# andrewhou1/GeomConsistentFR

Measured on AMD Instinct MI355X. Metric: ray_steps_per_sec, higher is better.
Workload: dtype f64+f32

## Files before the change

### geomconsistentfr_amd/csrc/gcfr_device.hpp

```cpp
#pragma once

#include <hip/hip_runtime.h>
#include <stdint.h>

namespace gcfr {

constexpr float kEps4 = 0.0001f;
constexpr float kMaskedDistance = 1000000.0f;

constexpr int kBufferRsrcWord3 = 0x00020000;

__device__ inline __amdgpu_buffer_rsrc_t make_rsrc(const void *p, int bytes)
{
    return __builtin_amdgcn_make_buffer_rsrc(const_cast<void *>(p), 0, bytes, kBufferRsrcWord3);
}
__device__ inline float buf_load_f32(__amdgpu_buffer_rsrc_t r, int byte_off)
{
    return __builtin_bit_cast(float, __builtin_amdgcn_raw_buffer_load_b32(r, byte_off, 0, 0));
}
__device__ inline uint32_t buf_load_u8(__amdgpu_buffer_rsrc_t r, int byte_off)
{
    return __builtin_amdgcn_raw_buffer_load_b8(r, byte_off, 0, 0);
}

struct Box {
    float x_lo, x_hi, y_lo, y_hi;
};
__device__ __host__ inline Box image_box(int H, int W)
{
    return Box{-(W / 2.0f), W - W / 2.0f - 1.0f, 1.0f - H / 2.0f, H / 2.0f};
}

struct LightCase {
    int xcase, ycase;
};
__device__ inline LightCase classify_light(float Cx, float Cy, const Box &bx)
{
    LightCase lc;
    lc.xcase = (Cx < bx.x_lo) ? 0 : (Cx <= bx.x_hi ? 1 : 2);
    lc.ycase = (Cy < bx.y_lo) ? 0 : (Cy <= bx.y_hi ? 1 : 2);
    return lc;
}

__device__ inline void end_point(float x, float y, float Cx, float Cy, const Box &bx, LightCase lc,
                                 float &Ex, float &Ey)
{
    const float m = (Cy - y) / ((Cx - x) + kEps4);
    const float ic = Cy - m * Cx;
    float ex, ey;
    if (lc.xcase == 1) {
        if (lc.ycase == 1) {
            ex = Cx;
            ey = Cy;
        } else {
            const float yb = (lc.ycase == 0) ? bx.y_lo : bx.y_hi;
            ex = (yb - ic) / (m + kEps4);
            ey = yb;
        }
    } else {
        const float xb = (lc.xcase == 0) ? bx.x_lo : bx.x_hi;
        const float Xy = m * xb + ic;
        if (lc.ycase == 1) {
            ex = xb;
            ey = Xy;
        } else {
            const float yb = (lc.ycase == 0) ? bx.y_lo : bx.y_hi;
            const float Yx = (yb - ic) / (m + kEps4);
            const float b = (Yx >= bx.x_lo && Yx <= bx.x_hi) ? 1.0f : 0.0f;
            const float nb = 1.0f - b;
            ex = Yx * b + xb * nb;
            ey = yb * b + Xy * nb;
        }
    }
    ex = (ex < bx.x_lo) ? bx.x_lo : ex;
    ex = (ex > bx.x_hi) ? bx.x_hi : ex;
    ey = (ey < bx.y_lo) ? bx.y_lo : ey;
    ey = (ey > bx.y_hi) ? bx.y_hi : ey;
    Ex = ex;
    Ey = ey;
}

__device__ inline float sqrt_rn_normal(float x)
{
#ifdef GCFR_R04_FIXED_COST
    return __builtin_sqrtf(x);
#endif
    const float s = __builtin_amdgcn_sqrtf(x);
    const int si = __builtin_bit_cast(int, s);
    const float s_dn = __builtin_bit_cast(float, si - 1), s_up = __builtin_bit_cast(float, si + 1);
    const float e_dn = __builtin_fmaf(-s_dn, s, x), e_up = __builtin_fmaf(-s_up, s, x);
    float o = (e_dn <= 0.0f) ? s_dn : s;
    o = (e_up > 0.0f) ? s_up : o;
    return o;
}

__device__ inline float norm3_torch(float a, float b, float c)
{
    return __builtin_sqrtf(__builtin_fmaf(c, c, __builtin_fmaf(b, b, a * a)));
}

__device__ inline float exp_neg(float d)
{
    const float x = -((d > 200.0f) ? 200.0f : d);
    const float kL2eHi = 1.44269502e+0f, kL2eLo = 1.92596299e-8f;
    const float t = x * kL2eHi;
    const float lo = __builtin_fmaf(x, kL2eLo, __builtin_fmaf(x, kL2eHi, -t));
    const float r = __builtin_amdgcn_exp2f(t);
    return __builtin_fmaf(r, lo * 0.693147182f, r);
}
__device__ inline float shadow_transfer(float d)
{
#ifdef GCFR_R04_FIXED_COST
    {
        const float e = expf(-d);
        const float onepe = 1.0f + e;
        return (-4.0f * e) / (onepe * onepe) + 1.0f;
    }
#endif
    const float e = exp_neg(d);
    const float onepe = 1.0f + e;
    const float q = onepe * onepe;
    float rq = __builtin_amdgcn_rcpf(q);
    rq = __builtin_fmaf(__builtin_fmaf(-q, rq, 1.0f), rq, rq);
    return (-4.0f * e) * rq + 1.0f;
}

struct Shaded {
    float w, full, fin;
};
__device__ inline float inv_norm3_clamped(float a, float b, float c)
{
    const float s2 = __builtin_fmaf(c, c, __builtin_fmaf(b, b, a * a));
    const float r = __builtin_amdgcn_rsqf(s2);
    const float r1 = r * __builtin_fmaf(-0.5f * s2 * r, r, 1.5f);
    return s2 > 1e-24f ? r1 : 1e12f;
}
__device__ inline float lambert_dot(float x, float y, float zb, float nx, float ny, float nz, float Cx, float Cy, float Cz)
{
    const float lx = Cx - x, ly = Cy - y, lz = Cz - zb;
#ifdef GCFR_R04_FIXED_COST
    {
        float ln = norm3_torch(lx, ly, lz);
        ln = ln > 1e-12f ? ln : 1e-12f;
        const float ux = lx / ln, uy = ly / ln, uz = lz / ln;
        float nn = norm3_torch(nx, ny, nz);
        nn = nn > 1e-12f ? nn : 1e-12f;
        const float n0 = nx / nn, n1 = ny / nn, n2 = nz / nn;
        return (n0 * ux + n1 * uy) + n2 * uz;
    }
#endif
    const float rl = inv_norm3_clamped(lx, ly, lz);
    const float ux = lx * rl, uy = ly * rl, uz = lz * rl;
    const float rn = inv_norm3_clamped(nx, ny, nz);
    const float n0 = nx * rn, n1 = ny * rn, n2 = nz * rn;
    return (n0 * ux + n1 * uy) + n2 * uz;
}

__device__ inline Shaded shade_pixel(float x, float y, float zb, float nx, float ny, float nz, float Cx,
                                     float Cy, float Cz, float amb, float intensity, float min_dist)
{
    const float dot = lambert_dot(x, y, zb, nx, ny, nz, Cx, Cy, Cz);
    Shaded o;
    o.full = amb + intensity * (dot > 0.0f ? dot : 0.0f);
    o.w = shadow_transfer(min_dist);
    o.fin = o.w * o.full + (1.0f - o.w) * amb;
    return o;
}

struct NormalsArgs {
    const float *depth;
    float *normals;
    const float *grad_normals;
    float *grad_depth;
    int32_t H, W;
    double fx, fy, cx, cy;
    float z_offset;
    int32_t negate_y;
    double inv_fx, inv_fy;
};
inline void set_focal(NormalsArgs &a, double fx, double fy)
{
    a.fx = fx;
    a.fy = fy;
    a.inv_fx = 1.0 / fx;
    a.inv_fy = 1.0 / fy;
}

__device__ constexpr double kSobelU[3][3] = {{-0.125, 0.0, 0.125}, {-0.25, 0.0, 0.25}, {-0.125, 0.0, 0.125}};
__device__ constexpr double kSobelV[3][3] = {{-0.125, -0.25, -0.125}, {0.0, 0.0, 0.0}, {0.125, 0.25, 0.125}};

struct Grad3 {
    double du[3], dv[3];
};

__device__ inline double fast_rcp64(double x)
{
    double r = __builtin_amdgcn_rcp(x);
    r = __builtin_fma(r, __builtin_fma(-x, r, 1.0), r);
    r = __builtin_fma(r, __builtin_fma(-x, r, 1.0), r);
    return r;
}

__device__ inline double fast_sqrt64(double x)
{
    double y = __builtin_amdgcn_rsq(x);
    double g = x * y, h = 0.5 * y;
    double e = __builtin_fma(-h, g, 0.5);
    g = __builtin_fma(g, e, g);
    h = __builtin_fma(h, e, h);
    e = __builtin_fma(-h, g, 0.5);
    g = __builtin_fma(g, e, g);
    return g;
}

__device__ inline Grad3 point_gradients(const NormalsArgs &a, const float *z, int r, int c)
{
    Grad3 g = {{0.0, 0.0, 0.0}, {0.0, 0.0, 0.0}};
    int rr[3], cc[3];
    double ax[3], ay[3];
#pragma unroll
    for (int j = 0; j < 3; ++j) {
        rr[j] = min(max(r + j - 1, 0), a.H - 1);
        cc[j] = min(max(c + j - 1, 0), a.W - 1);
        ax[j] = ((double)cc[j] - a.cx) * a.inv_fx;
        ay[j] = ((double)rr[j] - a.cy) * a.inv_fy;
    }
#pragma unroll
    for (int dr = -1; dr <= 1; ++dr) {
#pragma unroll
        for (int dc = -1; dc <= 1; ++dc) {
            const double d = (double)(z[(size_t)rr[dr + 1] * a.W + cc[dc + 1]] + a.z_offset);
            const double ku = kSobelU[dr + 1][dc + 1], kv = kSobelV[dr + 1][dc + 1];
            if (ku == 0.0 && kv == 0.0) {
                g.du[2] = __builtin_fma(0.0, d, g.du[2]);
                continue;
            }
            const double X = ax[dc + 1] * d, Y = ay[dr + 1] * d;
            if (ku != 0.0) {
                g.du[0] = __builtin_fma(ku, X, g.du[0]);
                g.du[1] = __builtin_fma(ku, Y, g.du[1]);
                g.du[2] = __builtin_fma(ku, d, g.du[2]);
            }
            if (kv != 0.0) {
                g.dv[0] = __builtin_fma(kv, X, g.dv[0]);
                g.dv[1] = __builtin_fma(kv, Y, g.dv[1]);
                g.dv[2] = __builtin_fma(kv, d, g.dv[2]);
            }
        }
    }
    return g;
}

__device__ inline double fast_rsqrt64(double x)
{
    const double y = __builtin_amdgcn_rsq(x);
    const double g = x * y, h = 0.5 * y;
    return __builtin_fma(y, __builtin_fma(-h, g, 0.5), y);
}

__device__ inline void unit_normal(const NormalsArgs &a, const float *z, int r, int c, float (&n)[3])
{
#ifdef GCFR_R04_FIXED_COST
    {
        const Grad3 g = point_gradients(a, z, r, c);
        const double nx = __builtin_fma(g.du[1], g.dv[2], -(g.du[2] * g.dv[1]));
        const double ny = __builtin_fma(g.du[2], g.dv[0], -(g.du[0] * g.dv[2]));
        const double nz = __builtin_fma(g.du[0], g.dv[1], -(g.du[1] * g.dv[0]));
        const double n2sum = __builtin_fma(nz, nz, __builtin_fma(ny, ny, nx * nx));
        double nn = n2sum > 1e-24 ? fast_sqrt64(n2sum) : 1e-12;
        nn = nn > 1e-12 ? nn : 1e-12;
        const double inv = fast_rcp64(nn);
        n[0] = (float)(nx * inv);
        n[1] = (float)(a.negate_y ? -(ny * inv) : (ny * inv));
        n[2] = (float)(nz * inv);
        return;
    }
#endif
    const int W = a.W;
    const bool has_l = c > 0, has_r = c < W - 1, has_u = r > 0, has_d = r < a.H - 1;
    const __amdgpu_buffer_rsrc_t zr = make_rsrc(z, a.H * W * 4);
    const int b11 = (r * W + c) << 2, W4 = W << 2;
    const int bu = has_u ? b11 - W4 : b11, bd = has_d ? b11 + W4 : b11;
    const int ol = has_l ? 4 : 0, orr = has_r ? 4 : 0;
    const float off = a.z_offset;
    const float D11 = buf_load_f32(zr, b11) + off;
    const float e00 = (buf_load_f32(zr, bu - ol) + off) - D11, e01 = (buf_load_f32(zr, bu) + off) - D11, e02 = (buf_load_f32(zr, bu + orr) + off) - D11;
    const float e10 = (buf_load_f32(zr, b11 - ol) + off) - D11, e12 = (buf_load_f32(zr, b11 + orr) + off) - D11;
    const float e20 = (buf_load_f32(zr, bd - ol) + off) - D11, e21 = (buf_load_f32(zr, bd) + off) - D11, e22 = (buf_load_f32(zr, bd + orr) + off) - D11;
    const float h0 = e02 - e00, h1 = e12 - e10, h2 = e22 - e20;
    const float g0 = e20 - e00, g1 = e21 - e01, g2 = e22 - e02;
    const float a8 = __builtin_fmaf(2.0f, h1, h0 + h2), b8 = __builtin_fmaf(2.0f, g1, g0 + g2);
    const float er = __builtin_fmaf(2.0f, e12, e02 + e22), el = __builtin_fmaf(2.0f, e10, e00 + e20);
    const float eb = __builtin_fmaf(2.0f, e21, e20 + e22), et = __builtin_fmaf(2.0f, e01, e00 + e02);
    const float s_x = (has_r ? er : 0.0f) + (has_l ? el : 0.0f), s_y = (has_d ? eb : 0.0f) + (has_u ? et : 0.0f);
    const float v_y = (has_d ? h2 : 0.0f) - (has_u ? h0 : 0.0f), v_x = (has_r ? g2 : 0.0f) - (has_l ? g0 : 0.0f);
    const float Dx = (has_l && has_r) ? D11 : 0.5f * D11, Dy = (has_u && has_d) ? D11 : 0.5f * D11;
    const double inv_fx = a.inv_fx, inv_fy = a.inv_fy;
    const double px = inv_fx * __builtin_fma(0.125, (double)s_x, (double)Dx), py = (0.125 * inv_fy) * (double)v_y;
    const double qx = (0.125 * inv_fx) * (double)v_x, qy = inv_fy * __builtin_fma(0.125, (double)s_y, (double)Dy);
    const double da = 0.125 * (double)a8, db = 0.125 * (double)b8;
    const double mx = __builtin_fma(da, qx, -(db * px)), my = __builtin_fma(da, qy, -(db * py));
    const double ax = ((double)c - a.cx) * inv_fx, ay = ((double)r - a.cy) * inv_fy;
    const double nx = -my, ny = mx;
    const double nz = __builtin_fma(ax, my, -(ay * mx)) + __builtin_fma(px, qy, -(py * qx));
    const double n2sum = __builtin_fma(nz, nz, __builtin_fma(ny, ny, nx * nx));
    const double inv = n2sum > 1e-24 ? fast_rsqrt64(n2sum) : 1e12;
    n[0] = (float)(nx * inv);
    n[1] = (float)(a.negate_y ? -(ny * inv) : (ny * inv));
    n[2] = (float)(nz * inv);
}

struct StencilGrad {
    double ddu[3], ddv[3];
};
__device__ inline StencilGrad normals_bwd_terms(const NormalsArgs &a, const float *z, int r, int c, double g0,
                                                double g1_in, double g2)
{
#pragma clang fp contract(fast)
    const Grad3 g = point_gradients(a, z, r, c);
    const double cx_ = g.du[1] * g.dv[2] - g.du[2] * g.dv[1];
    const double cy_ = g.du[2] * g.dv[0] - g.du[0] * g.dv[2];
    const double cz_ = g.du[0] * g.dv[1] - g.du[1] * g.dv[0];
    const double c2sum = cx_ * cx_ + cy_ * cy_ + cz_ * cz_;
    const double nrm = c2sum > 1e-24 ? fast_sqrt64(c2sum) : 0.0;
    const double nn = nrm > 1e-12 ? nrm : 1e-12;
    const double inv_nn = fast_rcp64(nn);
    const double n0 = cx_ * inv_nn, n1 = cy_ * inv_nn, n2 = cz_ * inv_nn;
    const double g1 = a.negate_y ? -g1_in : g1_in;
    double dc0, dc1, dc2;
    if (nrm > 1e-12) {
        const double ng = n0 * g0 + n1 * g1 + n2 * g2;
        dc0 = (g0 - n0 * ng) * inv_nn;
        dc1 = (g1 - n1 * ng) * inv_nn;
        dc2 = (g2 - n2 * ng) * inv_nn;
    } else {
        dc0 = g0 * inv_nn;
        dc1 = g1 * inv_nn;
        dc2 = g2 * inv_nn;
    }
    StencilGrad o;
    o.ddu[0] = g.dv[1] * dc2 - g.dv[2] * dc1;
    o.ddu[1] = g.dv[2] * dc0 - g.dv[0] * dc2;
    o.ddu[2] = g.dv[0] * dc1 - g.dv[1] * dc0;
    o.ddv[0] = dc1 * g.du[2] - dc2 * g.du[1];
    o.ddv[1] = dc2 * g.du[0] - dc0 * g.du[2];
    o.ddv[2] = dc0 * g.du[1] - dc1 * g.du[0];
    return o;
}

template <class Pred>
__device__ inline void normals_bwd_scatter(const NormalsArgs &a, const StencilGrad &sg, float *gz, int r, int c, Pred want)
{
#pragma clang fp contract(fast)
    const double inv_fx = a.inv_fx, inv_fy = a.inv_fy;
#pragma unroll
    for (int dr = -1; dr <= 1; ++dr) {
#pragma unroll
        for (int dc = -1; dc <= 1; ++dc) {
            const double ku = kSobelU[dr + 1][dc + 1], kv = kSobelV[dr + 1][dc + 1];
            if (ku == 0.0 && kv == 0.0)
                continue;
            if (!want(dr, dc))
                continue;
            const int rr = min(max(r + dr, 0), a.H - 1), cc = min(max(c + dc, 0), a.W - 1);
            const double ax = ((double)cc - a.cx) * inv_fx, ay = ((double)rr - a.cy) * inv_fy;
            const double dPx = ku * sg.ddu[0] + kv * sg.ddv[0];
            const double dPy = ku * sg.ddu[1] + kv * sg.ddv[1];
            const double dPz = ku * sg.ddu[2] + kv * sg.ddv[2];
#ifdef GCFR_ATOMIC_HOOK
            GCFR_ATOMIC_HOOK(gz + (size_t)rr * a.W + cc);
#endif
            atomicAdd(gz + (size_t)rr * a.W + cc, (float)(ax * dPx + ay * dPy + dPz));
        }
    }
}

__device__ inline void normals_bwd_pixel(const NormalsArgs &a, const float *z, float *gz, int r, int c,
                                         double g0, double g1_in, double g2)
{
    const StencilGrad sg = normals_bwd_terms(a, z, r, c, g0, g1_in, g2);
    normals_bwd_scatter(a, sg, gz, r, c, [](int, int) { return true; });
}

}
```

### geomconsistentfr_amd/csrc/gcfr_march.hpp

```cpp
#pragma once

#include "gcfr_device.hpp"
#include "gcfr_mutants.hpp"

#include "../../include/gcfr.h"

#include <atomic>
#include <cstddef>
#include <type_traits>

namespace gcfr {

struct ShadowArgs {
    const float *depth;
    const uint8_t *mask;
    const float *light_pt;
    const double *t_table;
    float *min_dist;
    int32_t *argmin;
    int32_t mask_batch, L, H, W, N;
    int32_t tiles_x, tiles_per_image;
    float bonus, bx_lo, bx_hi, by_lo, by_hi;
};

// ... 801 lines not shown
        ++cnt_since_body;
#endif
        const bool dead = OWN && (lane_last < 0);
        bool none = true;
#pragma unroll
        for (int j = 0; j < DEPTH; ++j) {
            none = none && (cm[j] == 0);
            any_masked |= (cm[j] == 0);
        }
        none = none || dead;
        bool run_body = __builtin_amdgcn_ballot_w64(!none) != 0ull;
        if (LAZY) {
            run_body = __builtin_amdgcn_ballot_w64(!none && !cw_in) != 0ull;
        } else if (run_body && use_zb) {
            const bool cannot_win = bound_cw(cz, ta64, tb64, k0);
            run_body = __builtin_amdgcn_ballot_w64(!none && !cannot_win) != 0ull;
            if (TRAIL)
                all_lazy = !run_body && __builtin_amdgcn_ballot_w64(!((cannot_win && GCFR_M(18, true, (bestS < safeS))) || (lane_last < k0))) == 0ull;
        }
#ifndef GCFR_INFER_BODY_CHUNK
#define GCFR_INFER_BODY_CHUNK 1
#endif
        constexpr int GCFR_BODY_CHUNK = KSPLIT ? DEPTH : (WANT_ARGMIN && DEPTH >= 2 ? 2 : GCFR_INFER_BODY_CHUNK);
        if (run_body) {
          GCFR_COUNT(kCntBodies, 1);
#ifdef GCFR_COUNTERS
          if (!cnt_had_body)
              cnt[kCntVisitsBeforeFirstBody] += cnt_since_body - 1;
          cnt_had_body = 1;
          cnt_since_body = 0;
#endif
#ifdef GCFR_COUNTERS
#pragma unroll
          for (int j = 0; j < DEPTH; ++j)
              cnt[kCntLaneSamples] += (unsigned)__builtin_popcountll(__builtin_amdgcn_ballot_w64(cm[j] != 0));
#endif
#pragma unroll
          for (int h0 = 0; h0 < DEPTH; h0 += GCFR_BODY_CHUNK) {
            double ux[DEPTH], uy[DEPTH], fxd[DEPTH], fyd[DEPTH];
            f32x4 qv[DEPTH];
#pragma unroll
            for (int j = h0; j < h0 + GCFR_BODY_CHUNK && j < DEPTH; ++j) {
                constexpr bool CARRIED = FUSE_SHADE || WANT_ARGMIN;
                const double tj = (CARRIED && j == 0) ? ta64 : ((CARRIED && j == DEPTH - 1) ? tb64 : (double)tt[clampk(k0 + j)]);
                const double sx = x64 + tj * dx64, sy = y64 + tj * dy64;
                ux[j] = (sx + halfW) - 0.0001;
                uy[j] = (halfH - sy) - 0.0001;
                fxd[j] = __builtin_floor(ux[j]);
                fyd[j] = __builtin_floor(uy[j]);
                const int fx = (int)fxd[j], fy = (int)fyd[j];
                const int texel = __mul24(fy, Wp) + fx;
                qv[j] = __builtin_bit_cast(
                    f32x4, __builtin_amdgcn_raw_buffer_load_b128(qr, (texel << 4) + quad_origin, 0, 0));
            }
#pragma unroll
            for (int j = h0; j < h0 + GCFR_BODY_CHUNK && j < DEPTH; ++j)
                eval_sample(clampk(k0 + j), (cm[j] == 0) || dead, ux[j], uy[j], fxd[j], fyd[j], qv[j]);
          }
        }
        return finish_check(k0, tn64, check_finished);
    };
    auto group = [&](int k0, const Prefetched &cur, Prefetched &nxt, bool check_finished) -> bool {
        const double ta64 = tc0, tb64 = tc3;
        tc0 = tq[0];
        tc3 = tq[DEPTH - 1];
        prefetch(nxt);
        load_tq(k0 + 2 * DEPTH);
        return consume(k0, cur.m, cur.z, ta64, tb64, tc0, check_finished, std::false_type{}, false);
    };

    auto group_lds = [&](int k0, bool check_finished) -> bool {
        const double ta64 = tq[0], tb64 = tq[DEPTH - 1];
        uint32_t cm[DEPTH];
        int cj[DEPTH], rj[DEPTH], cell[DEPTH];
        GCFR_COUNT(kCntGroupsVisited, 1);
        bool cw = false;
        if (use_zb) {
            double px, py;
            pos_tq(0, px, py);
            cell[0] = mask_offset(px, py, cj[0], rj[0]);
            pos_tq(DEPTH - 1, px, py);
            cell[DEPTH - 1] = mask_offset(px, py, cj[DEPTH - 1], rj[DEPTH - 1]);
            const f32x4 cz = lds_zb_fetch(cj[0], rj[0], cj[DEPTH - 1], rj[DEPTH - 1]);
            cw = bound_cw(cz, ta64, tb64, k0);
            if (__builtin_amdgcn_ballot_w64(!(cw && (bestS < safeS))) == 0ull) {
#ifdef GCFR_AUDIT
                audit_safe(cw);
#endif
                load_tq(k0 + DEPTH);
                return finish_check(k0, tq[0], check_finished);
            }
        }
        if (ALL_ONES) {
#pragma unroll
            for (int j = 0; j < DEPTH; ++j)
                cm[j] = 1u;
        } else {
#pragma unroll
            for (int j = 0; j < DEPTH; ++j) {
                if (!(use_zb && (j == 0 || j == DEPTH - 1))) {
                    double px, py;
                    pos_tq(j, px, py);
                    cell[j] = mask_offset(px, py, cj[j], rj[j]);
                }
                cm[j] = lds_load_b32((cell[j] >> 3) & ~3);
            }
        }
        load_tq(k0 + DEPTH);
        if (!ALL_ONES) {
#pragma unroll
            for (int j = 0; j < DEPTH; ++j)
                cm[j] = __builtin_amdgcn_ubfe(cm[j], (uint32_t)cj[j], 1u);
        }
        return consume(k0, cm, f32x4{}, ta64, tb64, tq[0], check_finished, std::true_type{}, cw);
    };

    if (LDS) {
        __syncthreads();
        if (k_begin < k_end)
            load_tq(k_begin);
        for (int k0 = k_begin; k0 < k_end; k0 += 2 * DEPTH) {
            if (!group_lds(k0, false))
                break;
            if (k0 + DEPTH >= k_end)
                break;
            if (!group_lds(k0 + DEPTH, true))
                break;
        }
    } else if (ROUGH) {
        constexpr int CH = WANT_ARGMIN ? GCFR_ROUGH_CHUNK_ARGMIN : GCFR_ROUGH_CHUNK;
        double tr[CH];
        auto load_tr = [&](int kfirst) {
#pragma unroll
            for (int j = 0; j < CH; ++j)
                tr[j] = tt[clampk(kfirst + j)];
        };
        if (k_begin < k_end)
            load_tr(k_begin);
        for (int k0 = k_begin; k0 < k_end; k0 += CH) {
            GCFR_COUNT(kCntRoughSamples, min(CH, k_end - k0));
            double ux[CH], uy[CH], fxd[CH], fyd[CH];
            f32x4 qv[CH];
            uint32_t mk[CH];
#pragma unroll
            for (int j = 0; j < CH; ++j) {
                const double tj = tr[j];
                const double sx = x64 + tj * dx64, sy = y64 + tj * dy64;
                int cr, rr;
                const int moff = mask_offset(sx, sy, cr, rr);
                mk[j] = ALL_ONES ? 1u : buf_load_u8(mr, moff);
                ux[j] = (sx + halfW) - 0.0001;
                uy[j] = (halfH - sy) - 0.0001;
                fxd[j] = __builtin_floor(ux[j]);
                fyd[j] = __builtin_floor(uy[j]);
                const int texel = __mul24((int)fyd[j], Wp) + (int)fxd[j];
                qv[j] = __builtin_bit_cast(f32x4, __builtin_amdgcn_raw_buffer_load_b128(qr, (texel << 4) + quad_origin, 0, 0));
            }
            load_tr(k0 + CH);
#pragma unroll
            for (int j = 0; j < CH; ++j) {
                const bool masked = (mk[j] == 0) || (OWN && (lane_last < 0));
                any_masked |= masked;
                eval_sample(clampk(k0 + j), masked, ux[j], uy[j], fxd[j], fyd[j], qv[j]);
            }
        }
    } else {
    Prefetched bufA, bufB;
    bufA.z = bufB.z = f32x4{0.0f, 0.0f, -__builtin_inff(), __builtin_inff()};
    const int k_first = k_begin;
    if (k_first < k_end) {
        load_tq(k_first);
        tc0 = tq[0];
        tc3 = tq[DEPTH - 1];
        prefetch(bufA);
        load_tq(k_first + DEPTH);
    }
    int k_trail = k_end;
    f32x4 zcur = bufA.z;
    for (int k0 = k_first; k0 < k_end; k0 += 2 * DEPTH) {
        if (!group(k0, bufA, bufB, false))
            break;
        if (k0 + DEPTH >= k_end)
            break;
        if (TRAIL && all_lazy) {
            k_trail = k0 + DEPTH;
            zcur = bufB.z;
            break;
        }
        if (!group(k0 + DEPTH, bufB, bufA, true))
            break;
        if (TRAIL && all_lazy && k0 + 2 * DEPTH < k_end) {
            k_trail = k0 + 2 * DEPTH;
            zcur = bufA.z;
            break;
        }
    }
    if (TRAIL) {
        if (k_trail < k_end)
            GCFR_COUNT(kCntTrailEnter, 1);
        auto record_of = [&](double t_first, double t_last) -> f32x4 {
            int ca, ra, cb, rb;
            (void)mask_offset(x64 + t_first * dx64, y64 + t_first * dy64, ca, ra);
            (void)mask_offset(x64 + t_last * dx64, y64 + t_last * dy64, cb, rb);
            return zb_fetch(ca, ra, cb, rb);
        };
        for (int k0 = k_trail; k0 < k_end; k0 += DEPTH) {
            const double ta64 = tc0, tb64 = tc3;
            tc0 = tq[0];
            tc3 = tq[DEPTH - 1];
            const f32x4 znext = record_of(tc0, tc3);
            load_tq(k0 + 2 * DEPTH);
            const bool check = (((k0 - k_trail) / DEPTH) & 1) != 0;
            const int hz_off = (GCFR_HORIZON != 0) && check && (k0 + DEPTH < k_end) ? launder(a)->hz_off : -1;
            const bool check_hz = hz_off >= 0;
            const float tn = (float)tc0;
            const bool cw = bound_cw(zcur, ta64, tb64, k0);
            const bool gone = lane_last < k0 GCFR_M(27, + 1, );
            GCFR_COUNT(kCntGroupsVisited, 1);
            if (__builtin_amdgcn_ballot_w64(!((cw && GCFR_M(18, true, (bestS < safeS))) || gone)) == 0ull) {
                any_masked |= gone;
                GCFR_COUNT(kCntTrailSkips, 1);
#ifdef GCFR_AUDIT
                audit_safe(cw && !gone);
                audit_masked(k0, min(k0 + DEPTH, k_end), gone);
#endif
#ifdef GCFR_COUNTERS
                ++cnt_since_body;
#endif
                if (check_hz) {
                    float dxl, dyl;
                    dir_f32(dxl, dyl);
                    const int ci = (int)__builtin_floorf(__builtin_fmaf(tn, dxl, x)), ri = (int)__builtin_floorf(-__builtin_fmaf(tn, dyl, y));
                    constexpr int C = kHorizonDim / 2, M = kHorizonDim - 1;
                    const int ic = (dxl >= 0.0f) ? kHorizonDim + min(max(ci + C, 0), M) : min(max(ci + C, 0), M);
                    const int ir = (dyl > 0.0f) ? 2 * kHorizonDim + min(max(ri + C, 0), M) : 3 * kHorizonDim + min(max(ri + C, 0), M);
                    const f32x4 zc4 = __builtin_bit_cast(f32x4, __builtin_amdgcn_raw_buffer_load_b128(zr, hz_off + (ic << 4), 0, 0));
                    const f32x4 zr4 = __builtin_bit_cast(f32x4, __builtin_amdgcn_raw_buffer_load_b128(zr, hz_off + (ir << 4), 0, 0));
                    const float zc = fmaxf(fmaxf(zc4.x, zc4.y), fmaxf(zc4.z, zc4.w)), zr_ = fmaxf(fmaxf(zr4.x, zr4.y), fmaxf(zr4.z, zr4.w));
                    float nrm_l = nrm;
                    asm volatile("" : "+v"(nrm_l));
                    const float Dc = __builtin_fmaf(nrm_l, fminf(zc, zr_), -(nrm_l * zb)) + Kerr;
                    const float gd = __builtin_fmaf(c1, tn, -Dc);
                    const bool past = lane_last < k0 + DEPTH GCFR_M(26, + 1, );
                    const bool finished = (GCFR_M(11, true, (c1 > 0.0f)) && (gd > 0.0f) && (gd * gd * GCFR_M(8, GCFR_MUT_SLACK_VALUE, 0.998f) > bestS) && (bestS < safeS)) || past;
                    if (__builtin_amdgcn_ballot_w64(!finished) == 0ull) {
                        any_masked |= past;
                        GCFR_COUNT(kCntEarlyExit, 1);
#ifdef GCFR_AUDIT
                        audit_finish(k0 + DEPTH, GCFR_M(11, true, (c1 > 0.0f)) && (gd > 0.0f) && (gd * gd * GCFR_M(8, GCFR_MUT_SLACK_VALUE, 0.998f) > bestS) && (bestS < safeS),
                                     gd, GCFR_M(8, GCFR_MUT_SLACK_VALUE, 0.998f), past);
#endif
                        break;
                    }
                } else if (!finish_check(k0, tc0, check)) {
                    break;
                }
            } else {
                GCFR_COUNT(kCntTrailLeave, 1);
                uint32_t cm[DEPTH];
#pragma unroll
                for (int j = 0; j < DEPTH; ++j) {
                    const double tj = (j == 0) ? ta64 : ((j == DEPTH - 1) ? tb64 : (double)tt[clampk(k0 + j)]);
                    int cj, rj;
                    cm[j] = ALL_ONES ? 1u : buf_load_u8(mr, mask_offset(x64 + tj * dx64, y64 + tj * dy64, cj, rj));
                }
                if (!consume(k0, cm, zcur, ta64, tb64, tc0, check, std::true_type{}, cw))
                    break;
                zcur = record_of(tc0, tc3);
                continue;
            }
            zcur = znext;
        }
    }
    }

    if (KSPLIT) {
        __shared__ float sS[4][64], sPS[4][64];
        __shared__ int sK[4][64], sPK[4][64];
        __shared__ uint8_t sM[4][64];
        sS[wave][lane] = bestS;
        sK[wave][lane] = besti;
        sPS[wave][lane] = prevS;
        sPK[wave][lane] = prevk;
        sM[wave][lane] = any_masked ? 1 : 0;
        __syncthreads();
        if (wave != 0)
            return false;
#pragma unroll
        for (int q = 1; q < 4; ++q) {
            const float Sq = sS[q][lane];
            const bool take = Sq < bestS;
            const float PSq = sPS[q][lane];
            const bool local_pred = PSq < bestS;
            prevS = take ? (local_pred ? PSq : bestS) : prevS;
            prevk = take ? (local_pred ? sPK[q][lane] : besti) : prevk;
            bestS = take ? Sq : bestS;
            besti = take ? sK[q][lane] : besti;
            any_masked |= (sM[q][lane] != 0);
        }
    }

    float BCx_e = BCx;
    asm volatile("" : "+v"(BCx_e));
    const float den = sqrt_rn_normal(((BCx_e * BCx_e + BCy * BCy) + BCz * BCz) + kEps4);
    float d = sqrt_rn_normal(bestS) / den;
    if (WANT_ARGMIN) {
        const bool tie = GCFR_M(16, false &&, ) (prevk >= 0) && (sqrt_rn_normal(prevS) / den == d);
        if (__builtin_amdgcn_ballot_w64(tie) != 0ull) {
            GCFR_COUNT(kCntTieRemarch, 1);
            RayConst rc;
            rc.H = H;
            rc.W = W;
            rc.halfW = halfW;
            rc.halfH = halfH;
            rc.x = x;
            rc.y = y;
            rc.zb = zb;
            dir_f32(rc.dx, rc.dy);
            rc.BCx = BCx;
            rc.BCy = BCy;
            rc.BCz = BCz;
            rc.x64 = x64;
            rc.y64 = y64;
            rc.dx64 = dx64;
            rc.dy64 = dy64;
            const int first = first_tied_sample(rc, a->t_table, make_rsrc(a->depth + (size_t)b * P, (int)(P * 4)), mr,
                                                tie, prevk, den, d);
            besti = tie ? first : besti;
        }
    }
    if (any_masked && !(d < kMaskedDistance)) {
        d = kMaskedDistance;
        besti = -1;
    }
    if (OWN && (lane_last < 0)) {
        d = kMaskedDistance;
        besti = -1;
    }
    if (!finite_ray)
        d = __builtin_nanf("");
    const EpiPtr ep = launder((EpiPtr)&a->epi);
    const bool inside = (Cx >= ep->bx_lo) && (Cx <= ep->bx_hi) && (Cy >= ep->by_lo) && (Cy <= ep->by_hi);
    if (inside)
        d = d + ep->bonus;
    {
        const int lane_e = fresh_lane_id();
        const int r_e = qy * TILE_H + lane_e / TILE_W, c_e = tx * TILE_W + (lane_e % TILE_W);
        const bool valid_e = (r_e < H) && (c_e < W);
        r = valid_e ? r_e : H - 1;
        c = valid_e ? c_e : W - 1;
        if (!valid_e)
            return false;
    }
    {
        const size_t pix = (size_t)r * W + c;
        const size_t o = (size_t)bl * P + pix;
        ep->min_dist[o] = d;
        if (WANT_ARGMIN)
            ep->argmin[o] = besti;
        if (FUSE_SHADE) {
            float n[3];
            const float *normals = ep->normals;
            if (normals) {
                const float *nrm = normals + (size_t)b * 3 * P + pix;
                n[0] = nrm[0];
                n[1] = nrm[P];
                n[2] = nrm[2 * P];
            } else {
                NormalsArgs na = {};
                na.H = H;
                na.W = W;
                na.inv_fx = ep->nrm.inv_fx;
                na.inv_fy = ep->nrm.inv_fy;
                na.cx = ep->nrm.cx;
                na.cy = ep->nrm.cy;
                na.z_offset = ep->nrm.z_offset;
                na.negate_y = ep->nrm.negate_y;
                unit_normal(na, a->depth + (size_t)b * P, r, c, n);
                float *normals_out = ep->normals_out;
                if (normals_out && l == 0) {
                    float *no = normals_out + (size_t)b * 3 * P + pix;
                    no[0] = n[0];
                    no[P] = n[1];
                    no[2 * P] = n[2];
                }
            }
            const Shaded sh = shade_pixel(x, y, zb, n[0], n[1], n[2], Cx, Cy, Cz, ep->ambient[bl], ep->intensity, d);
            float *shadow_w = ep->shadow_w, *full = ep->full, *final_shading = ep->final_shading;
            if (shadow_w)
                shadow_w[o] = sh.w;
            if (full)
                full[o] = sh.full;
            if (final_shading)
                final_shading[o] = sh.fin;
            const float *alb = ep->albedo + (size_t)b * 3 * P + pix;
            float *ren = ep->rendered + (size_t)bl * 3 * P + pix;
#pragma unroll
            for (int ch = 0; ch < 3; ++ch)
                ren[ch * P] = alb[ch * P] * sh.fin;
        }
    }
#ifdef GCFR_COUNTERS
    if (a->counters && lane == 0 && !(KSPLIT && wave != 0)) {
        cnt[kCntVisitsAfterLastBody] += cnt_since_body;
#ifndef GCFR_TRACE_ONLY
#pragma unroll
        for (int i = 0; i < kCntUsed; ++i) {
            if (i == kCntAuditMaxUse)
                atomicMax(a->counters + i, (unsigned long long)cnt[i]);
            else
                atomicAdd(a->counters + i, (unsigned long long)cnt[i]);
        }
#endif
        unsigned long long *rec = a->counters + GCFR_N_COUNTERS + 4 * ((size_t)(bl * a->tiles_y + qy) * a->tiles_x + tx);
        const unsigned hw_id = __builtin_amdgcn_s_getreg((31 << 11) | 4);
        const unsigned xcc_id = __builtin_amdgcn_s_getreg((31 << 11) | 20);
        rec[0] = trace_t0;
        rec[1] = __builtin_amdgcn_s_memrealtime();
        rec[2] = __builtin_amdgcn_s_memtime() - trace_c0;
        rec[3] = (unsigned long long)hw_id | ((unsigned long long)(xcc_id & 0xf) << 32) |
                 ((unsigned long long)(cnt[kCntBodies] & 0xfff) << 36) | ((unsigned long long)(cnt[kCntGroupsVisited] & 0xfff) << 48);
    }
#endif
    return false;
}

#ifndef GCFR_MARCH_WAVES_PER_EU
#define GCFR_MARCH_WAVES_PER_EU 6
#endif
#ifndef GCFR_MARCH_ARGMIN_WAVES_PER_EU
#define GCFR_MARCH_ARGMIN_WAVES_PER_EU 5
#endif

template <int TILE_W, bool EVEN_HALF, bool WANT_ARGMIN, int DEPTH, bool FUSE_SHADE, bool LDS = false, bool OWN = false>
__device__ __forceinline__ void march_grid(ArgPtr a)
{
    const int wave = __builtin_amdgcn_readfirstlane((int)(threadIdx.x >> 6));
    const int tx = (int)blockIdx.x * 4 + wave;
    const int bl = a->bl_offset + (int)blockIdx.z;
    const bool want_z = (a->zb != nullptr);
    const ImageStats st = reduce_image_stats(a, bl / a->L, threadIdx.x & 63, want_z);
    if (LDS)
        stage_lds(a, bl / a->L, st.mask_all_ones == 0);
    if (tx >= a->tiles_x) {
        if (LDS)
            __syncthreads();
        return;
    }
    constexpr int FULL = (LDS || GCFR_ROUGH == 0) ? kModeInline : kModeFull;
    bool rough;
    if (st.mask_all_ones != 0)
        rough = march_tile<TILE_W, EVEN_HALF, WANT_ARGMIN, DEPTH, FUSE_SHADE, 0, true, LDS, false, FULL>(a, bl, (int)blockIdx.y, tx, st);
    else
        rough = march_tile<TILE_W, EVEN_HALF, WANT_ARGMIN, DEPTH, FUSE_SHADE, 0, false, LDS, OWN, FULL>(a, bl, (int)blockIdx.y, tx, st);
    if (FULL == kModeFull && GCFR_M(15, false &&, ) __builtin_amdgcn_readfirstlane((int)rough) != 0) {
        const ArgPtr a2 = WANT_ARGMIN ? a : launder(a);
        const int bl2 = WANT_ARGMIN ? bl : a2->bl_offset + (int)blockIdx.z;
        const ImageStats st2 = WANT_ARGMIN ? st : reduce_image_stats(a2, bl2 / a2->L, threadIdx.x & 63, false);
        if (st2.mask_all_ones != 0)
            march_tile<TILE_W, EVEN_HALF, WANT_ARGMIN, DEPTH, FUSE_SHADE, 0, true, false, false, kModeRough>(a2, bl2, (int)blockIdx.y, tx, st2);
        else
            march_tile<TILE_W, EVEN_HALF, WANT_ARGMIN, DEPTH, FUSE_SHADE, 0, false, false, OWN, kModeRough>(a2, bl2, (int)blockIdx.y, tx, st2);
    }
}

enum { kSchedGrid = 0 };

template <int SCHED, int TILE_W, bool EVEN_HALF, bool WANT_ARGMIN, int DEPTH, bool FUSE_SHADE, bool LDS = false, bool OWN = false>
__device__ __forceinline__ void march_dispatch()
{
    static_assert(SCHED == kSchedGrid, "the product library has the grid schedule only");
    march_grid<TILE_W, EVEN_HALF, WANT_ARGMIN, DEPTH, FUSE_SHADE, LDS, OWN>(kernel_args());
}

template <int TILE_W, bool EVEN_HALF, int DEPTH, bool FUSE_SHADE, int SCHED>
__global__ __launch_bounds__(256)
__attribute__((amdgpu_waves_per_eu(GCFR_MARCH_WAVES_PER_EU, GCFR_MARCH_WAVES_PER_EU))) void shadow_fwd_quad_kernel(ShadowQuadArgs)
{
    march_dispatch<SCHED, TILE_W, EVEN_HALF, false, DEPTH, FUSE_SHADE>();
}
template <int TILE_W, bool EVEN_HALF, int DEPTH, bool FUSE_SHADE, int SCHED>
__global__ __launch_bounds__(256)
__attribute__((amdgpu_waves_per_eu(GCFR_MARCH_ARGMIN_WAVES_PER_EU, GCFR_MARCH_ARGMIN_WAVES_PER_EU))) void shadow_fwd_quad_argmin_kernel(ShadowQuadArgs)
{
    march_dispatch<SCHED, TILE_W, EVEN_HALF, true, DEPTH, FUSE_SHADE>();
}
template <int TILE_W, bool EVEN_HALF, int DEPTH, bool FUSE_SHADE, int SCHED>
__global__ __launch_bounds__(256)
__attribute__((amdgpu_waves_per_eu(GCFR_MARCH_ARGMIN_WAVES_PER_EU, GCFR_MARCH_ARGMIN_WAVES_PER_EU))) void shadow_fwd_quad_argmin_own_kernel(ShadowQuadArgs)
{
    march_dispatch<SCHED, TILE_W, EVEN_HALF, true, DEPTH, FUSE_SHADE, false, true>();
}
template <int TILE_W, bool EVEN_HALF, int DEPTH, bool FUSE_SHADE, int SCHED>
__global__ __launch_bounds__(256)
__attribute__((amdgpu_waves_per_eu(GCFR_MARCH_WAVES_PER_EU, GCFR_MARCH_WAVES_PER_EU))) void shadow_fwd_quad_lds_kernel(ShadowQuadArgs)
{
    march_dispatch<SCHED, TILE_W, EVEN_HALF, false, DEPTH, FUSE_SHADE, true>();
}
template <int TILE_W, bool EVEN_HALF, int DEPTH, bool FUSE_SHADE, int SCHED>
__global__ __launch_bounds__(256)
__attribute__((amdgpu_waves_per_eu(GCFR_MARCH_ARGMIN_WAVES_PER_EU, GCFR_MARCH_ARGMIN_WAVES_PER_EU))) void shadow_fwd_quad_argmin_lds_kernel(ShadowQuadArgs)
{
    march_dispatch<SCHED, TILE_W, EVEN_HALF, true, DEPTH, FUSE_SHADE, true>();
}
template <int TILE_W, bool EVEN_HALF, bool WANT_ARGMIN, int DEPTH, bool FUSE_SHADE>
__global__ __launch_bounds__(256) void shadow_fwd_quad_ksplit_kernel(ShadowQuadArgs)
{
    const ArgPtr a = kernel_args();
    const int bl = a->bl_offset + (int)blockIdx.z;
    const ImageStats st = reduce_image_stats(a, bl / a->L, threadIdx.x & 63, a->zb != nullptr);
    march_tile<TILE_W, EVEN_HALF, WANT_ARGMIN, DEPTH, FUSE_SHADE, 1>(a, bl, (int)blockIdx.y, (int)blockIdx.x, st);
}


enum Schedule { kGrid = kSchedGrid, kKSplit, kGridLds, kGridOwn };

template <int TILE_W, int DEPTH, bool FUSE>
static void launch_quad4(const ShadowQuadArgs &a, bool even_half, bool want_argmin, Schedule sch, dim3 grid,
                         hipStream_t st, unsigned lds_bytes)
{
#define GCFR_LAUNCH(KERNEL, ...) hipLaunchKernelGGL((KERNEL<TILE_W, __VA_ARGS__>), grid, dim3(256), 0, st, a)
#define GCFR_LAUNCH_LDS(KERNEL, ...) hipLaunchKernelGGL((KERNEL<TILE_W, __VA_ARGS__>), grid, dim3(256), lds_bytes, st, a)
#define GCFR_LAUNCH_SCHED(SCHED)                                                    \
    do {                                                                            \
        if (even_half) {                                                            \
            if (want_argmin)                                                        \
                GCFR_LAUNCH(shadow_fwd_quad_argmin_kernel, true, DEPTH, FUSE, SCHED);  \
            else                                                                    \
                GCFR_LAUNCH(shadow_fwd_quad_kernel, true, DEPTH, FUSE, SCHED);      \
        } else {                                                                    \
            if (want_argmin)                                                        \
                GCFR_LAUNCH(shadow_fwd_quad_argmin_kernel, false, DEPTH, FUSE, SCHED); \
            else                                                                    \
                GCFR_LAUNCH(shadow_fwd_quad_kernel, false, DEPTH, FUSE, SCHED);     \
        }                                                                           \
    } while (0)
    if (sch == kKSplit) {
        if (even_half) {
            if (want_argmin)
                GCFR_LAUNCH(shadow_fwd_quad_ksplit_kernel, true, true, DEPTH, FUSE);
            else
                GCFR_LAUNCH(shadow_fwd_quad_ksplit_kernel, true, false, DEPTH, FUSE);
        } else {
            if (want_argmin)
                GCFR_LAUNCH(shadow_fwd_quad_ksplit_kernel, false, true, DEPTH, FUSE);
            else
                GCFR_LAUNCH(shadow_fwd_quad_ksplit_kernel, false, false, DEPTH, FUSE);
        }
    } else if (sch == kGridLds) {
        if constexpr (TILE_W == 16 && DEPTH == 4) {
            if (even_half) {
                if (want_argmin)
                    GCFR_LAUNCH_LDS(shadow_fwd_quad_argmin_lds_kernel, true, DEPTH, FUSE, kSchedGrid);
                else
                    GCFR_LAUNCH_LDS(shadow_fwd_quad_lds_kernel, true, DEPTH, FUSE, kSchedGrid);
            } else {
                if (want_argmin)
                    GCFR_LAUNCH_LDS(shadow_fwd_quad_argmin_lds_kernel, false, DEPTH, FUSE, kSchedGrid);
                else
                    GCFR_LAUNCH_LDS(shadow_fwd_quad_lds_kernel, false, DEPTH, FUSE, kSchedGrid);
            }
        }
    } else if (sch == kGridOwn) {
        if (even_half)
            GCFR_LAUNCH(shadow_fwd_quad_argmin_own_kernel, true, DEPTH, FUSE, kSchedGrid);
        else
            GCFR_LAUNCH(shadow_fwd_quad_argmin_own_kernel, false, DEPTH, FUSE, kSchedGrid);
    } else {
        GCFR_LAUNCH_SCHED(kSchedGrid);
    }
#undef GCFR_LAUNCH_SCHED
#undef GCFR_LAUNCH_LDS
#undef GCFR_LAUNCH
}

template <int TILE_W, int DEPTH>
static void launch_quad3(const ShadowQuadArgs &a, bool even_half, bool want_argmin, Schedule sch, dim3 grid,
                         hipStream_t st, unsigned lds_bytes)
{
    if (a.epi.rendered)
        launch_quad4<TILE_W, DEPTH, true>(a, even_half, want_argmin, sch, grid, st, lds_bytes);
    else
        launch_quad4<TILE_W, DEPTH, false>(a, even_half, want_argmin, sch, grid, st, lds_bytes);
}

typedef void (*MarchUnitFn)(const ShadowQuadArgs &a, bool even_half, bool want_argmin, Schedule sch, dim3 grid,
                            hipStream_t st, unsigned lds_bytes);
#define GCFR_MARCH_UNIT_NAME_(TW, G) launch_march_##TW##_##G
#define GCFR_MARCH_UNIT_NAME(TW, G) GCFR_MARCH_UNIT_NAME_(TW, G)
#define GCFR_DECLARE_MARCH_UNIT(TW, G)                                                                              \
    void GCFR_MARCH_UNIT_NAME(TW, G)(const ShadowQuadArgs &a, bool even_half, bool want_argmin, Schedule sch, dim3 grid, \
                                     hipStream_t st, unsigned lds_bytes);
GCFR_DECLARE_MARCH_UNIT(16, 4)
#ifndef GCFR_FAST_BUILD
GCFR_DECLARE_MARCH_UNIT(16, 2)
GCFR_DECLARE_MARCH_UNIT(16, 1)
GCFR_DECLARE_MARCH_UNIT(8, 4)
GCFR_DECLARE_MARCH_UNIT(8, 2)
GCFR_DECLARE_MARCH_UNIT(8, 1)
GCFR_DECLARE_MARCH_UNIT(32, 4)
GCFR_DECLARE_MARCH_UNIT(32, 2)
GCFR_DECLARE_MARCH_UNIT(32, 1)
GCFR_DECLARE_MARCH_UNIT(64, 4)
GCFR_DECLARE_MARCH_UNIT(64, 2)
GCFR_DECLARE_MARCH_UNIT(64, 1)
#endif

}
```

Baseline: 2359 billion.

## Prefetch epilogue depth stencil and albedo early; use nontemporal output stores

The epilogue's parameter loads, the 3x3 depth stencil used for the normal, and the albedo reads are moved ahead of the tie re-march and the distance computation, so their memory latency overlaps that work. The normal computation is split into a stencil load part and a compute part so the loads can be issued early. Output stores become nontemporal when argmin is not requested, to avoid polluting the cache. The cost is higher register pressure across the tie path, and invalid lanes now issue loads they previously skipped.

```diff
diff --git a/geomconsistentfr_amd/csrc/gcfr_device.hpp b/geomconsistentfr_amd/csrc/gcfr_device.hpp
--- a/geomconsistentfr_amd/csrc/gcfr_device.hpp
+++ b/geomconsistentfr_amd/csrc/gcfr_device.hpp
@@ -258,35 +258,27 @@
     return __builtin_fma(y, __builtin_fma(-h, g, 0.5), y);
 }
 
-__device__ inline void unit_normal(const NormalsArgs &a, const float *z, int r, int c, float (&n)[3])
-{
-#ifdef GCFR_R04_FIXED_COST
-    {
-        const Grad3 g = point_gradients(a, z, r, c);
-        const double nx = __builtin_fma(g.du[1], g.dv[2], -(g.du[2] * g.dv[1]));
-        const double ny = __builtin_fma(g.du[2], g.dv[0], -(g.du[0] * g.dv[2]));
-        const double nz = __builtin_fma(g.du[0], g.dv[1], -(g.du[1] * g.dv[0]));
-        const double n2sum = __builtin_fma(nz, nz, __builtin_fma(ny, ny, nx * nx));
-        double nn = n2sum > 1e-24 ? fast_sqrt64(n2sum) : 1e-12;
-        nn = nn > 1e-12 ? nn : 1e-12;
-        const double inv = fast_rcp64(nn);
-        n[0] = (float)(nx * inv);
-        n[1] = (float)(a.negate_y ? -(ny * inv) : (ny * inv));
-        n[2] = (float)(nz * inv);
-        return;
-    }
-#endif
-    const int W = a.W;
-    const bool has_l = c > 0, has_r = c < W - 1, has_u = r > 0, has_d = r < a.H - 1;
-    const __amdgpu_buffer_rsrc_t zr = make_rsrc(z, a.H * W * 4);
+__device__ inline void load_depth_stencil(int H, int W, const float *z, int r, int c, float (&v)[9])
+{
+    const bool has_l = c > 0, has_r = c < W - 1, has_u = r > 0, has_d = r < H - 1;
+    const __amdgpu_buffer_rsrc_t zr = make_rsrc(z, H * W * 4);
     const int b11 = (r * W + c) << 2, W4 = W << 2;
     const int bu = has_u ? b11 - W4 : b11, bd = has_d ? b11 + W4 : b11;
     const int ol = has_l ? 4 : 0, orr = has_r ? 4 : 0;
+    v[4] = buf_load_f32(zr, b11);
+    v[0] = buf_load_f32(zr, bu - ol), v[1] = buf_load_f32(zr, bu), v[2] = buf_load_f32(zr, bu + orr);
+    v[3] = buf_load_f32(zr, b11 - ol), v[5] = buf_load_f32(zr, b11 + orr);
+    v[6] = buf_load_f32(zr, bd - ol), v[7] = buf_load_f32(zr, bd), v[8] = buf_load_f32(zr, bd + orr);
+}
+__device__ inline void unit_normal_from(const NormalsArgs &a, const float (&v)[9], int r, int c, float (&n)[3])
+{
+    const int W = a.W;
+    const bool has_l = c > 0, has_r = c < W - 1, has_u = r > 0, has_d = r < a.H - 1;
     const float off = a.z_offset;
-    const float D11 = buf_load_f32(zr, b11) + off;
-    const float e00 = (buf_load_f32(zr, bu - ol) + off) - D11, e01 = (buf_load_f32(zr, bu) + off) - D11, e02 = (buf_load_f32(zr, bu + orr) + off) - D11;
-    const float e10 = (buf_load_f32(zr, b11 - ol) + off) - D11, e12 = (buf_load_f32(zr, b11 + orr) + off) - D11;
-    const float e20 = (buf_load_f32(zr, bd - ol) + off) - D11, e21 = (buf_load_f32(zr, bd) + off) - D11, e22 = (buf_load_f32(zr, bd + orr) + off) - D11;
+    const float D11 = v[4] + off;
+    const float e00 = (v[0] + off) - D11, e01 = (v[1] + off) - D11, e02 = (v[2] + off) - D11;
+    const float e10 = (v[3] + off) - D11, e12 = (v[5] + off) - D11;
+    const float e20 = (v[6] + off) - D11, e21 = (v[7] + off) - D11, e22 = (v[8] + off) - D11;
     const float h0 = e02 - e00, h1 = e12 - e10, h2 = e22 - e20;
     const float g0 = e20 - e00, g1 = e21 - e01, g2 = e22 - e02;
     const float a8 = __builtin_fmaf(2.0f, h1, h0 + h2), b8 = __builtin_fmaf(2.0f, g1, g0 + g2);
@@ -309,6 +301,28 @@
     n[1] = (float)(a.negate_y ? -(ny * inv) : (ny * inv));
     n[2] = (float)(nz * inv);
 }
+__device__ inline void unit_normal(const NormalsArgs &a, const float *z, int r, int c, float (&n)[3])
+{
+#ifdef GCFR_R04_FIXED_COST
+    {
+        const Grad3 g = point_gradients(a, z, r, c);
+        const double nx = __builtin_fma(g.du[1], g.dv[2], -(g.du[2] * g.dv[1]));
+        const double ny = __builtin_fma(g.du[2], g.dv[0], -(g.du[0] * g.dv[2]));
+        const double nz = __builtin_fma(g.du[0], g.dv[1], -(g.du[1] * g.dv[0]));
+        const double n2sum = __builtin_fma(nz, nz, __builtin_fma(ny, ny, nx * nx));
+        double nn = n2sum > 1e-24 ? fast_sqrt64(n2sum) : 1e-12;
+        nn = nn > 1e-12 ? nn : 1e-12;
+        const double inv = fast_rcp64(nn);
+        n[0] = (float)(nx * inv);
+        n[1] = (float)(a.negate_y ? -(ny * inv) : (ny * inv));
+        n[2] = (float)(nz * inv);
+        return;
+    }
+#endif
+    float v[9];
+    load_depth_stencil(a.H, a.W, z, r, c, v);
+    unit_normal_from(a, v, r, c, n);
+}
 
 struct StencilGrad {
     double ddu[3], ddv[3];
diff --git a/geomconsistentfr_amd/csrc/gcfr_march.hpp b/geomconsistentfr_amd/csrc/gcfr_march.hpp
--- a/geomconsistentfr_amd/csrc/gcfr_march.hpp
+++ b/geomconsistentfr_amd/csrc/gcfr_march.hpp
@@ -1127,6 +1127,51 @@
 
     float BCx_e = BCx;
     asm volatile("" : "+v"(BCx_e));
+    const int lane_e = fresh_lane_id();
+    const int r_e = qy * TILE_H + lane_e / TILE_W, c_e = tx * TILE_W + (lane_e % TILE_W);
+    const bool valid_e = (r_e < H) && (c_e < W);
+    r = valid_e ? r_e : H - 1;
+    c = valid_e ? c_e : W - 1;
+    const size_t pix = (size_t)r * W + c;
+    const size_t o = (size_t)bl * P + pix;
+    const EpiPtr ep = launder((EpiPtr)&a->epi);
+    float *const min_dist = ep->min_dist;
+    int32_t *const argmin = WANT_ARGMIN ? ep->argmin : nullptr;
+    const float bonus = ep->bonus, bx_lo = ep->bx_lo, bx_hi = ep->bx_hi, by_lo = ep->by_lo, by_hi = ep->by_hi;
+    const float *const normals = FUSE_SHADE ? ep->normals : nullptr;
+    const float *const albedo = FUSE_SHADE ? ep->albedo : nullptr;
+    float *const shadow_w = FUSE_SHADE ? ep->shadow_w : nullptr, *const full = FUSE_SHADE ? ep->full : nullptr;
+    float *const final_shading = FUSE_SHADE ? ep->final_shading : nullptr, *const rendered = FUSE_SHADE ? ep->rendered : nullptr;
+    float *const normals_out = FUSE_SHADE ? ep->normals_out : nullptr;
+    const float intensity = FUSE_SHADE ? ep->intensity : 0.0f;
+    const float amb = FUSE_SHADE ? ((ConstF32Ptr)(unsigned long long)ep->ambient)[bl] : 0.0f;
+    NormalsArgs na = {};
+    float zs[9], n[3], alb[3];
+    if (FUSE_SHADE) {
+        na.H = H;
+        na.W = W;
+        na.inv_fx = ep->nrm.inv_fx;
+        na.inv_fy = ep->nrm.inv_fy;
+        na.cx = ep->nrm.cx;
+        na.cy = ep->nrm.cy;
+        na.z_offset = ep->nrm.z_offset;
+        na.negate_y = ep->nrm.negate_y;
+        if (normals) {
+            const float *nrm_in = normals + (size_t)b * 3 * P + pix;
+            n[0] = nrm_in[0];
+            n[1] = nrm_in[P];
+            n[2] = nrm_in[2 * P];
+        } else {
+#ifndef GCFR_R04_FIXED_COST
+            load_depth_stencil(H, W, a->depth + (size_t)b * P, r, c, zs);
+#endif
+        }
+        const float *alb_in = albedo + (size_t)b * 3 * P + pix;
+#pragma unroll
+        for (int ch = 0; ch < 3; ++ch)
+            alb[ch] = alb_in[ch * P];
+    }
+
     const float den = sqrt_rn_normal(((BCx_e * BCx_e + BCy * BCy) + BCz * BCz) + kEps4);
     float d = sqrt_rn_normal(bestS) / den;
     if (WANT_ARGMIN) {
@@ -1164,66 +1209,48 @@
     }
     if (!finite_ray)
         d = __builtin_nanf("");
-    const EpiPtr ep = launder((EpiPtr)&a->epi);
-    const bool inside = (Cx >= ep->bx_lo) && (Cx <= ep->bx_hi) && (Cy >= ep->by_lo) && (Cy <= ep->by_hi);
+    const bool inside = (Cx >= bx_lo) && (Cx <= bx_hi) && (Cy >= by_lo) && (Cy <= by_hi);
     if (inside)
-        d = d + ep->bonus;
-    {
-        const int lane_e = fresh_lane_id();
-        const int r_e = qy * TILE_H + lane_e / TILE_W, c_e = tx * TILE_W + (lane_e % TILE_W);
-        const bool valid_e = (r_e < H) && (c_e < W);
-        r = valid_e ? r_e : H - 1;
-        c = valid_e ? c_e : W - 1;
-        if (!valid_e)
-            return false;
-    }
-    {
-        const size_t pix = (size_t)r * W + c;
-        const size_t o = (size_t)bl * P + pix;
-        ep->min_dist[o] = d;
-        if (WANT_ARGMIN)
-            ep->argmin[o] = besti;
-        if (FUSE_SHADE) {
-            float n[3];
-            const float *normals = ep->normals;
-            if (normals) {
-                const float *nrm = normals + (size_t)b * 3 * P + pix;
-                n[0] = nrm[0];
-                n[1] = nrm[P];
-                n[2] = nrm[2 * P];
-            } else {
-                NormalsArgs na = {};
-                na.H = H;
-                na.W = W;
-                na.inv_fx = ep->nrm.inv_fx;
-                na.inv_fy = ep->nrm.inv_fy;
-                na.cx = ep->nrm.cx;
-                na.cy = ep->nrm.cy;
-                na.z_offset = ep->nrm.z_offset;
-                na.negate_y = ep->nrm.negate_y;
-                unit_normal(na, a->depth + (size_t)b * P, r, c, n);
-                float *normals_out = ep->normals_out;
-                if (normals_out && l == 0) {
-                    float *no = normals_out + (size_t)b * 3 * P + pix;
-                    no[0] = n[0];
-                    no[P] = n[1];
-                    no[2 * P] = n[2];
-                }
+        d = d + bonus;
+    if (!valid_e)
+        return false;
+#ifndef GCFR_EPI_NT
+#define GCFR_EPI_NT 1
+#endif
+    auto store = [](auto *p, auto v) {
+        if ((GCFR_EPI_NT != 0) && !WANT_ARGMIN)
+            __builtin_nontemporal_store(v, p);
+        else
+            *p = v;
+    };
+    store(min_dist + o, d);
+    if (WANT_ARGMIN)
+        store(argmin + o, besti);
+    if (FUSE_SHADE) {
+        if (!normals) {
+#ifdef GCFR_R04_FIXED_COST
+            unit_normal(na, a->depth + (size_t)b * P, r, c, n);
+#else
+            unit_normal_from(na, zs, r, c, n);
+#endif
+            if (normals_out && l == 0) {
+                float *no = normals_out + (size_t)b * 3 * P + pix;
+                store(no, n[0]);
+                store(no + P, n[1]);
+                store(no + 2 * P, n[2]);
             }
-            const Shaded sh = shade_pixel(x, y, zb, n[0], n[1], n[2], Cx, Cy, Cz, ep->ambient[bl], ep->intensity, d);
-            float *shadow_w = ep->shadow_w, *full = ep->full, *final_shading = ep->final_shading;
-            if (shadow_w)
-                shadow_w[o] = sh.w;
-            if (full)
-                full[o] = sh.full;
-            if (final_shading)
-                final_shading[o] = sh.fin;
-            const float *alb = ep->albedo + (size_t)b * 3 * P + pix;
-            float *ren = ep->rendered + (size_t)bl * 3 * P + pix;
-#pragma unroll
-            for (int ch = 0; ch < 3; ++ch)
-                ren[ch * P] = alb[ch * P] * sh.fin;
-        }
+        }
+        const Shaded sh = shade_pixel(x, y, zb, n[0], n[1], n[2], Cx, Cy, Cz, amb, intensity, d);
+        if (shadow_w)
+            store(shadow_w + o, sh.w);
+        if (full)
+            store(full + o, sh.full);
+        if (final_shading)
+            store(final_shading + o, sh.fin);
+        float *ren = rendered + (size_t)bl * 3 * P + pix;
+#pragma unroll
+        for (int ch = 0; ch < 3; ++ch)
+            store(ren + ch * P, alb[ch] * sh.fin);
     }
 #ifdef GCFR_COUNTERS
     if (a->counters && lane == 0 && !(KSPLIT && wave != 0)) {
```

After: 2441 billion (median of 6 runs). 1.04x the previous value.
